# bghira/universal-metal-flash-attention

Hardware: AMD Instinct MI355X
Metric: SDPA fwd TFLOPS (bf16) + int8 speedup, B=1 H=24 S=4096 D=128, 1/2/4/8 GPU (higher is better)
Workload: dtype bf16

## Files before the change

universal-metal-flash-attention_amd/csrc/fa_fwd16_w64.hip:

```cpp
#include <algorithm>
#include <cmath>
#include <cstdlib>
#include <type_traits>

#include "fa_fwd16_w64_params.h"

namespace umfa {

#define W64_I8 0
#define W64_BODY_INC "fa_fwd16_w64_body.inc"
#define W64_T __bf16
#define W64_MFMA "v_mfma_f32_32x32x16_bf16"
#define W64_MFMA_QK "v_mfma_f32_32x32x16_bf16"
#define W64_MSUM "v_mfma_f32_4x4x4_16b_bf16"
#define W64_ONES_BITS 0x3f803f80u
#define W64_LAZY_PARTS 1
#define W64_CVT "v_cvt_pk_bf16_f32"
#define W64_KERNEL fa_fwd16_w64_bf16
#include "fa_fwd16_w64_kernel.inc"
#undef W64_T
#undef W64_MFMA
#undef W64_MFMA_QK
#undef W64_MSUM
#undef W64_ONES_BITS
// ... 317 lines not shown
        const uint64_t items = (uint64_t)p.B * p.H * ((p.Sq + 255) / 256);
        const uint64_t cus = (uint64_t)w64_cu_count();
        if (const int gi = tuning().w64_grid.load(std::memory_order_relaxed)) {
            if (gi > 0 && (uint64_t)gi <= cus && (uint64_t)gi <= items && gi <= 512) return (uint32_t)gi;
        }
        const uint64_t gmax = cus < 512 ? cus : 512;
        if (items < cus) return (uint32_t)((p.ms[2] == 0 && items * ((p.Skv + 63) / 64) >= cus * 10) ? gmax : items);
        return (uint32_t)gmax;
    }
    const bool pairs = p.causal && !w64_is_window(p);
    uint64_t total = (uint64_t)p.B * p.H * ((p.Sq + 255) / 256) * w64_tiles_per_item(p);
    if (pairs) total = (uint64_t)p.B * p.H * (((p.Sq + 255) / 256 + 1) / 2);
    const uint32_t cus = (uint32_t)w64_cu_count();
    if (const int gi = tuning().w64_grid.load(std::memory_order_relaxed)) {
        const uint32_t g = (uint32_t)gi;
        if (gi > 0 && g <= cus && g <= total) return g;
    }
    if (!pairs) {
        const uint64_t items = (uint64_t)p.B * p.H * ((p.Sq + 255) / 256);
        if (items < cus && cus / items >= 2 && items * (cus / items) <= total) return (uint32_t)(items * (cus / items));
        if (items < cus && 2 * (uint64_t)w64_tiles_per_item(p) * (cus - items) < 35 * cus) return (uint32_t)items;
    }
    return total < cus ? (uint32_t)total : cus;
}

uint32_t fwd_w64_grid(const FwdParams& p) { return w64_grid(p); }

FwdW64Plan fwd_w64_plan(const FwdParams& p) {
    FwdW64Plan plan;
    const uint32_t items = p.B * p.H * ((p.Sq + 255) / 256);
    (void)items;
    plan.cnt_bytes = ((size_t)w64_grid(p) * sizeof(uint32_t) + 255) & ~(size_t)255;
    plan.buf_bytes = (size_t)2 * w64_grid(p) * (4 * 2 * 17 * 1024);
    return plan;
}

template <typename KFN>
static hipError_t launch_w64_kernel(KFN kfn, const FwdParams& p, const W64Params& wp, hipStream_t stream) {
    const uint32_t grid = w64_grid(p);
    const size_t lds = 65536 + 4 * 32 * (512 + 16) + 64 + 4096 + 8192 + 2048 + 64;
    if (hipError_t e = ensure_dynamic_lds((const void*)kfn, lds); e != hipSuccess) return e;
    hipLaunchKernelGGL(kfn, dim3(grid), dim3(256), lds, stream, wp);
    return hipGetLastError();
}

hipError_t launch_fwd_w64(const FwdParams& p, float* part_buf, uint32_t* part_cnt, hipStream_t stream, const char** name) {
    if (!fwd_w64_supported(p) || !part_buf || !part_cnt) return hipErrorNotSupported;
    W64Params wp;
    wp.q = p.q; wp.k = p.k; wp.v = p.v; wp.o = p.o; wp.lse = p.lse;
    for (int i = 0; i < 3; ++i) { wp.qs[i] = p.qs[i]; wp.ks[i] = p.ks[i]; wp.vs[i] = p.vs[i]; }
    wp.B = p.B; wp.H = p.H; wp.Sq = p.Sq; wp.Skv = p.Skv;
    wp.scale = p.scale;
    wp.n_items = p.B * p.H * ((p.Sq + 255) / 256);
    wp.T = (p.Skv + 63) / 64;
    wp.part_buf = part_buf;
    wp.part_cnt = part_cnt;
    w64_softmax_policy(p.in_prec, &wp.tau, &wp.lazy);
    wp.skew = (uint32_t)tuning().w64_skew.load(std::memory_order_relaxed);
    if (tuning().w64_skew.load(std::memory_order_relaxed) == -1) wp.skew = 0xffffffffu;
    wp.rope_cos = p.rope_cos; wp.rope_sin = p.rope_sin; wp.rope_tb = p.rope_tb;
    wp.vsc = p.vsc; wp.vsc_bs = p.vsc_bs; wp.vsc_hs = p.vsc_hs;
    if (p.in_prec == P_BF16 && p.pv16 && !p.vsc) return hipErrorInvalidValue;
    wp.Tw = wp.T; wp.win_left = wp.win_right = 0;
    const bool rope = p.rope_cos != nullptr, window = w64_is_window(p), fp32o = p.out_prec == P_FP32, maska = p.mask_kind == MK_F16, maskt = p.mask_kind == MK_BOOL || maska;
    wp.mask = nullptr; wp.mask_s[0] = wp.mask_s[1] = wp.mask_s[2] = 0;
    wp.guard = maska ? p.guard : nullptr;
    if (p.guard && (!maska || p.guard_want != 0u)) return hipErrorInvalidValue;
    if (maskt) {
        if ((!maska && !p.mk_bits) || !p.mk_list || !p.mk_cnt) return hipErrorInvalidValue;
        if (maska) { wp.mask = p.mask; wp.mask_s[0] = p.ms[0]; wp.mask_s[1] = p.ms[1]; wp.mask_s[2] = p.ms[2]; }
        wp.mk_bits = p.mk_bits; wp.mk_list = p.mk_list; wp.mk_cnt = p.mk_cnt;
        wp.mk_bs = p.mk_bs; wp.mk_hs = p.mk_hs; wp.mk_nrb64 = p.mk_nrb64;
        wp.mk_prefix = p.mk_prefix;
#ifndef W64_LAB_MASK_FORCE_LAZY
        if (p.ms[2] != 0 || p.causal || tuning().no_w64_mask_lazy.load(std::memory_order_relaxed)) wp.lazy = 0;
#endif
    }
    if (rope && p.out_prec != p.in_prec) return hipErrorNotSupported;
    if (window) {
        wp.Tw = w64_tiles_per_item(p);
        wp.win_left = (int32_t)w64_win_left(p);
        wp.win_right = (int32_t)w64_win_right(p);
    }
#define W64_FAMILY(FAM, T16, HAS_ROPE)                                                                                         \
    do {                                                                                                                       \
        if constexpr (HAS_ROPE >= 2) {        \
            if (maskt) return fp32o ? launch_w64_kernel(FAM<float, false, false, false, true>, p, wp, stream) : launch_w64_kernel(FAM<T16, false, false, false, true>, p, wp, stream); \
        }                                                                                                                      \
        if constexpr (HAS_ROPE == 1 || HAS_ROPE == 2) {                                                                        \
            if (rope) return p.causal ? launch_w64_kernel(FAM<T16, true, true>, p, wp, stream) : launch_w64_kernel(FAM<T16, false, true>, p, wp, stream); \
        }                                                                                                                      \
        if (window) return fp32o ? launch_w64_kernel(FAM<float, false, false, true>, p, wp, stream) : launch_w64_kernel(FAM<T16, false, false, true>, p, wp, stream); \
        if (p.causal) return fp32o ? launch_w64_kernel(FAM<float, true>, p, wp, stream) : launch_w64_kernel(FAM<T16, true>, p, wp, stream); \
        return fp32o ? launch_w64_kernel(FAM<float, false>, p, wp, stream) : launch_w64_kernel(FAM<T16, false>, p, wp, stream); \
    } while (0)
    static const char* const names[3][2][3] = {
        {{"fa_fwd16_w64<bf16,128>", "fa_fwd16_w64<bf16,128,rope>", "fa_fwd16_w64<bf16,128,window>"},
         {"fa_fwd16_w64<bf16,64>", "fa_fwd16_w64<bf16,64,rope>", "fa_fwd16_w64<bf16,64,window>"}},
        {{"fa_fwd16_w64<bf16,128,pv16>", "fa_fwd16_w64<bf16,128,pv16,rope>", "fa_fwd16_w64<bf16,128,pv16,window>"},
         {"fa_fwd16_w64<bf16,64,pv16>", "fa_fwd16_w64<bf16,64,pv16,rope>", "fa_fwd16_w64<bf16,64,pv16,window>"}},
        {{"fa_fwd16_w64<fp16,128>", "fa_fwd16_w64<fp16,128,rope>", "fa_fwd16_w64<fp16,128,window>"},
         {"fa_fwd16_w64<fp16,64>", "fa_fwd16_w64<fp16,64,rope>", "fa_fwd16_w64<fp16,64,window>"}}};
    if (p.D == 64 && rope) return hipErrorNotSupported;
    const int fam = p.in_prec == P_BF16 ? (p.pv16 ? 1 : 0) : 2;
    if (maskt && fam == 0) return hipErrorNotSupported;
    if (maska && fam == 0) return hipErrorNotSupported;
    if (maska) {
        *name = p.D == 64 ? (fam == 1 ? "fa_fwd16_w64<bf16,64,pv16,bias>" : "fa_fwd16_w64<fp16,64,bias>") : (fam == 1 ? "fa_fwd16_w64<bf16,128,pv16,bias>" : "fa_fwd16_w64<fp16,128,bias>");
        return launch_fwd_w64_bias(wp, fam, fp32o, w64_grid(p), 65536 + 4 * 32 * (512 + 16) + 64 + 4096 + 8192 + 2048 + 64, stream, (int)p.D);
    }
    *name = maska ? (fam == 1 ? "fa_fwd16_w64<bf16,128,pv16,bias>" : "fa_fwd16_w64<fp16,128,bias>") : maskt ? (p.D == 64 ? (fam == 1 ? "fa_fwd16_w64<bf16,64,pv16,mask>" : "fa_fwd16_w64<fp16,64,mask>")
                               : (fam == 1 ? "fa_fwd16_w64<bf16,128,pv16,mask>" : "fa_fwd16_w64<fp16,128,mask>"))
                  : names[fam][p.D == 64 ? 1 : 0][rope ? 1 : window ? 2 : 0];
    if (p.D == 64) {
        if (fam == 0) W64_FAMILY(fa_fwd16_w64d64_bf16, __bf16, 0);
        if (fam == 1) W64_FAMILY(fa_fwd16_w64d64_bf16pv16, __bf16, 3);
        W64_FAMILY(fa_fwd16_w64d64_f16, _Float16, 3);
    }
    if (fam == 0) W64_FAMILY(fa_fwd16_w64_bf16, __bf16, 1);
    if (fam == 1) W64_FAMILY(fa_fwd16_w64_bf16pv16, __bf16, 2);
    W64_FAMILY(fa_fwd16_w64_f16, _Float16, 2);
#undef W64_FAMILY
}

bool fwd_w64_i8_supported(const FwdParams& p) {
    if (tuning().no_w64.load(std::memory_order_relaxed) || p.D != 128) return false;
    if (!(p.scale > 0.0f)) return false;
    if (p.Skv < 64 || p.Sq < 256 || (p.Sq % 256 != 0 && p.Sq < 1024)) return false;
    if (p.mask_kind == MK_BOOL && p.mask) {
        if (tuning().no_w64_mask.load(std::memory_order_relaxed) || p.causal) return false;
        if (((p.Skv + 63) / 64) > 1024u || w64_grid(p) > 512u) return false;
        if (tuning().force_w64.load(std::memory_order_relaxed)) return true;
        const uint64_t blocks = (uint64_t)p.B * p.H * ((p.Sq + 255) / 256), cus = (uint64_t)w64_cu_count();
        return blocks >= cus || (p.ms[2] == 0 && blocks * ((p.Skv + 63) / 64) >= cus * 10) || ((p.ms[0] != 0 || p.ms[1] != 0) && blocks * 8 >= cus * 3);
    }
    return p.mask_kind == MK_NONE && !p.mask;
}

hipError_t launch_fwd_w64_i8(const FwdParams& p, const QuantViews& v, float* part_buf, uint32_t* part_cnt, hipStream_t stream) {
    if (!fwd_w64_i8_supported(p) || !part_buf || !part_cnt || v.dpq != 128) return hipErrorNotSupported;
    W64I8Params wp;
    wp.q8 = v.q8; wp.k8 = v.k8; wp.v16 = (const _Float16*)v.v16;
    wp.v8 = v.v8; wp.v_e8 = v.v_e8;
    wp.q_scale = v.q_scale; wp.k_scale = v.k_scale;
    wp.o = p.o; wp.lse = p.lse;
    wp.B = p.B; wp.H = p.H; wp.Sq = p.Sq; wp.Skv = p.Skv; wp.nqblk = v.nqblk; wp.nkblk = v.nkblk;
    wp.scale = p.scale;
    wp.n_items = p.B * p.H * ((p.Sq + 255) / 256);
    wp.T = (p.Skv + 63) / 64;
    wp.part_buf = part_buf;
    wp.part_cnt = part_cnt;
    w64_softmax_policy(P_FP16, &wp.tau, &wp.lazy);
    wp.skew = (uint32_t)tuning().w64_skew.load(std::memory_order_relaxed);
    wp.vsc = v.v8 ? nullptr : p.vsc;
    const uint32_t grid = w64_grid(p);
    const bool f8 = v.v8 != nullptr, maskt = p.mask_kind == MK_BOOL;
    wp.mk_bits = wp.mk_list = wp.mk_cnt = nullptr; wp.mk_bs = wp.mk_hs = wp.mk_nrb64 = 0;
    if (maskt) {
        if (f8 || p.causal || !p.mk_bits || !p.mk_list || !p.mk_cnt) return hipErrorInvalidValue;
        wp.mk_bits = p.mk_bits; wp.mk_list = p.mk_list; wp.mk_cnt = p.mk_cnt;
        wp.mk_bs = p.mk_bs; wp.mk_hs = p.mk_hs; wp.mk_nrb64 = p.mk_nrb64;
        if (p.ms[2] != 0 || tuning().no_w64_mask_lazy.load(std::memory_order_relaxed)) wp.lazy = 0;
    }
    const size_t lds = maskt ? 65536 + 4 * 32 * (512 + 16) + 64 + 4096 + 8192 + 2048 + 64 : 65536 + 4 * 32 * (512 + 16) + 16;
    auto kfn = f8 ? (p.causal ? fa_fwd_w64_i8f8<float, true> : fa_fwd_w64_i8f8<float, false>)
                  : maskt ? fa_fwd_w64_i8<float, false, true>
                          : (p.causal ? fa_fwd_w64_i8<float, true> : fa_fwd_w64_i8<float, false>);
    if (hipError_t e = ensure_dynamic_lds((const void*)kfn, lds); e != hipSuccess) return e;
    hipLaunchKernelGGL(kfn, dim3(grid), dim3(256), lds, stream, wp);
    return hipGetLastError();
}

}
```

universal-metal-flash-attention_amd/csrc/fa_fwd16_w64_kernel.inc:

```

#ifdef W64_ABL_NOBAR
#define W64_ITER_BARRIER() asm volatile("" ::: "memory")
#elif defined(W64_LAB_WAITSTAMP)
#define W64_ITER_BARRIER()                                                                         \
    do {                                                                                           \
        asm volatile("s_waitcnt lgkmcnt(0)" ::: "memory");                                         \
        const unsigned long long w0_ = __builtin_amdgcn_s_memtime();                               \
        asm volatile("s_waitcnt vmcnt(0) lgkmcnt(0)" ::: "memory");                                \
        const unsigned long long w1_ = __builtin_amdgcn_s_memtime();                               \
        asm volatile("s_waitcnt lgkmcnt(0)\n\ts_barrier" ::: "memory");                            \
        const unsigned long long w2_ = __builtin_amdgcn_s_memtime();                               \
        asm volatile("s_waitcnt lgkmcnt(0)" ::: "memory");                                         \
        st_wait += w1_ - w0_;                                                                      \
        st_bar += w2_ - w1_;                                                                       \
    } while (0)
#elif defined(W64_ABL_VMCNT8)
#define W64_ITER_BARRIER() asm volatile("s_waitcnt vmcnt(8) lgkmcnt(0)\n\ts_barrier" ::: "memory")
#else
#define W64_ITER_BARRIER() asm volatile("s_waitcnt vmcnt(0) lgkmcnt(0)\n\ts_barrier" ::: "memory")
#endif
#ifdef W64_ABL_NODMA
#define W64_DMA_ON 0
#else
#define W64_DMA_ON 1
// ... 138 lines not shown
    auto v_frag = [&](int voff, int db, int st) -> V8 {
        const V4 lo = tr_read_at(vtr[db] + (unsigned)(voff + (16 * st) * ROW_IN));
        const V4 hi4 = tr_read_at(vtr[db] + (unsigned)(voff + (16 * st + 8) * ROW_IN));
        return __builtin_shufflevector(lo, hi4, 0, 1, 2, 3, 4, 5, 6, 7);
    };
    (void)v_frag;

#if W64_F8
    typedef int i32x8 __attribute__((ext_vector_type(8)));
    const unsigned v8addr = lds0 + (unsigned)lane * 16u;
    auto v8_frag = [&](int voff, int db) -> i32x8 {
        const i32x4 lo = *(const i32x4 LDS_AS*)(uintptr_t)(v8addr + (unsigned)(voff + db * 2048));
        const i32x4 hi4 = *(const i32x4 LDS_AS*)(uintptr_t)(v8addr + (unsigned)(voff + db * 2048 + 1024));
        return __builtin_shufflevector(lo, hi4, 0, 1, 2, 3, 4, 5, 6, 7);
    };
#endif

#if W64_I8
    const int k_stride_b = 128, v_stride_b = 256, q_stride_b = 128;
#else
    const int k_stride_b = (int)p.ks[2] * 2, v_stride_b = (int)p.vs[2] * 2, q_stride_b = (int)p.qs[2] * 2;
#endif
    int kdma0[4], vdma0[4];
    {
        constexpr int RPI = 1024 / ROW_IN, CPR = ROW_IN / 16, PPW = 16 / RPI;
        const int d_r = lane / CPR, d_c = lane % CPR;
        (void)d_c;
#pragma unroll
        for (int j = 0; j < 4; ++j) {
            const int row = (uw * PPW + (j % PPW)) * RPI + d_r;
            (void)row;
#if W64_F8
            vdma0[j] = ((uw * 2 + (j & 1)) * 64 + lane) * 16;
#else
            vdma0[j] = row * v_stride_b + (v_off<W64_DP>(row, d_c) - row * ROW_IN);
#endif
#if W64_I8
            const int krow = (uw * 2 + (j & 1)) * 8 + (lane >> 3), kc = lane & 7;
            kdma0[j] = krow * 128 + (k8_off_128(krow, kc) - krow * 128);
#else
            kdma0[j] = row * k_stride_b + (k_off<W64_DP>(row, d_c) - row * ROW_IN);
#endif
        }
    }
    const int k_step0 = 64 * k_stride_b, v_step0 = W64_F8 ? 8192 : 64 * v_stride_b;
    const unsigned lds_wave = __builtin_amdgcn_readfirstlane(lds0 + (unsigned)uw * (W64_F8 ? 2048u : (unsigned)(16 * ROW_IN)));
#if W64_I8
    const unsigned lds_wave_k = __builtin_amdgcn_readfirstlane(lds0 + (unsigned)uw * 2048u);
    float c2 = 0.0f;
#ifndef W64_I8_NOBIAS
    constexpr float I8_BIAS = 12582912.0f;
#if W64_F8
    f8_init_consts();
#else
    i8_init_bias();
#endif
    float nmb[2] = {0.f, 0.f};
#endif
#else
    const unsigned lds_wave_k = lds_wave;
    const float c2 = p.scale * UMFA_LOG2E;
#endif

    const uint32_t G = gridDim.x;
    const uint32_t w = xcd_remap(blockIdx.x, G);
    const uint32_t T_ = p.T;
    const uint32_t nqb = (p.Sq + 255) / 256;
    const bool ktail = (p.Skv & 63) != 0;
    const uint32_t jobs_per_head = (nqb + 1) / 2, n_jobs = p.B * p.H * jobs_per_head;
    uint32_t Tst = T_;
    int win_left = 0, win_right = 0;
#if !W64_I8
    if constexpr (WINDOW) { Tst = p.Tw; win_left = p.win_left; win_right = p.win_right; }
#endif
    (void)win_left; (void)win_right;
    constexpr bool SPARSE = CAUSAL || WINDOW || MASKT;
    auto mk_slab = [&](uint32_t bh_) -> uint32_t { return (bh_ / p.H) * p.mk_bs + (bh_ % p.H) * p.mk_hs; };
    auto item_tiles = [&](uint32_t item) -> uint32_t {
        if constexpr (MASKT) return p.mk_cnt[mk_slab(item / nqb) * nqb + item % nqb];
        if constexpr (!CAUSAL) return Tst;
        const uint32_t q = item % nqb;
        return 4 * q + 4 < T_ ? 4 * q + 4 : T_;
    };
    const bool whole_rem = !CAUSAL && p.skew == 0xffffffffu;
    const uint32_t full_rounds = CAUSAL ? 0u : whole_rem ? (p.n_items + G - 1) / G : p.n_items / G;
    const uint32_t rem_items = (CAUSAL || whole_rem) ? 0u : p.n_items - full_rounds * G;
    constexpr unsigned MK_PREFIX_OFF = 65536u + 4u * 32u * (512u + 16u) + 64u + 4096u + 8192u;
    if constexpr (MASKT) {
        if (rem_items) {
            volatile uint32_t* const pf = (volatile uint32_t*)(smem + MK_PREFIX_OFF);
            const uint32_t first = full_rounds * G, j0 = threadIdx.x, j1 = threadIdx.x + 256u;
            for (uint32_t j = threadIdx.x; j < rem_items; j += 256u) {
                const uint32_t it_ = first + j;
                pf[1 + j] = p.mk_cnt[mk_slab(it_ / nqb) * nqb + it_ % nqb];
            }
            if (threadIdx.x == 0) pf[0] = 0u;
            __syncthreads();
            for (uint32_t off = 1; off < rem_items; off <<= 1) {
                const uint32_t a0 = (j0 < rem_items && j0 >= off) ? pf[1 + j0 - off] : 0u;
                const uint32_t a1 = (j1 < rem_items && j1 >= off) ? pf[1 + j1 - off] : 0u;
                __syncthreads();
                if (j0 < rem_items) pf[1 + j0] += a0;
                if (j1 < rem_items) pf[1 + j1] += a1;
                __syncthreads();
            }
        }
    }
    auto mk_prefix_at = [&](uint32_t j) -> uint32_t {
        return (uint32_t)__builtin_amdgcn_readfirstlane((int)((volatile const uint32_t*)(smem + MK_PREFIX_OFF))[j]);
    };
    (void)mk_prefix_at;
    auto item_start = [&](uint32_t litem) -> uint64_t {
        if constexpr (MASKT) return mk_prefix_at(litem);
        return (uint64_t)litem * Tst;
    };
    auto item_of_step = [&](uint64_t step) -> uint32_t {
        if constexpr (MASKT) {
            uint32_t lo = 0, hi_ = rem_items - 1;
            while (lo < hi_) {
                const uint32_t mid = (lo + hi_ + 1) >> 1;
                if (mk_prefix_at(mid) <= step) lo = mid; else hi_ = mid - 1;
            }
            return lo;
        }
        return (uint32_t)(step / Tst);
    };
    const uint64_t total = MASKT ? (rem_items ? (uint64_t)mk_prefix_at(rem_items) : 0ull) : (uint64_t)rem_items * Tst;
    const uint32_t skew = (!MASKT && rem_items && G == 2 * rem_items && p.skew != 0xffffffffu && 2 * p.skew < Tst) ? p.skew : 0u;
    const uint32_t Gs = (MASKT && total < G) ? (uint32_t)total : G;
    auto slice_bound = [&](uint32_t g) -> uint32_t {
        if constexpr (MASKT) { if (g >= Gs) return (uint32_t)total; }
        return (uint32_t)(total * g / Gs) - ((g & 1u) ? skew : 0u);
    };
    const uint32_t s_begin = slice_bound(w), s_end = slice_bound(w + 1);
#ifdef W64_LAB_GAPSTAMP
    unsigned long long st_g[4] = {0, 0, 0, 0}, st_gprev = 0;
#define W64_GSTAMP(k)                                                                            \
    do {                                                                                         \
        asm volatile("s_waitcnt lgkmcnt(0)" ::: "memory");                                       \
        const unsigned long long now_ = __builtin_amdgcn_s_memtime();                            \
        asm volatile("s_waitcnt lgkmcnt(0)" ::: "memory");                                       \
        if (st_gprev) st_g[k] += now_ - st_gprev;                                                \
        st_gprev = now_;                                                                         \
    } while (0)
#endif
#ifdef W64_LAB_FSTAMP
    unsigned long long fs_now[8] = {0, 0, 0, 0, 0, 0, 0, 0};
    uint32_t fs_acc[8] = {0, 0, 0, 0, 0, 0, 0, 0}, fs_last = 0, fs_tiles = 0;
    bool fs_valid = false;
#define W64_FSTAMP(k) asm volatile("s_memtime %0" : "=s"(fs_now[k]))
#define W64_FSTAMP_END(n)                                                                           \
    do {                                                                                            \
        asm volatile("s_waitcnt lgkmcnt(0)" ::: "memory");                                          \
        if (fs_valid) fs_acc[0] += (uint32_t)fs_now[0] - fs_last;                                   \
        _Pragma("unroll") for (int k_ = 1; k_ < (n); ++k_) fs_acc[k_] += (uint32_t)fs_now[k_] - (uint32_t)fs_now[k_ - 1]; \
        fs_last = (uint32_t)fs_now[(n) - 1];                                                        \
        fs_valid = true;                                                                            \
        ++fs_tiles;                                                                                 \
    } while (0)
#endif
#ifdef W64_LAB_STAMPS
    const unsigned long long st_rt0 = __builtin_amdgcn_s_memrealtime(), st_ck0 = __builtin_amdgcn_s_memtime();
    unsigned long long st_pro = 0, st_loop = 0, st_drain = 0, st_epi = 0, st_t = 0, st_wait = 0, st_bar = 0;
#define W64_STAMP(acc) do { const unsigned long long now_ = __builtin_amdgcn_s_memtime(); acc += now_ - st_t; st_t = now_; } while (0)
#else
#define W64_STAMP(acc) do { } while (0)
#endif

    uint32_t ntail = 0;
    bool tail_first = false;
    if (s_end > s_begin) {
        const uint32_t it0 = item_of_step(s_begin), it1 = item_of_step(s_end - 1);
        ntail = it1 - it0 + 1;
        tail_first = item_start(it0) != s_begin;
    }
    const uint32_t my_jobs = CAUSAL ? (n_jobs > w ? (n_jobs - w + G - 1) / G : 0u) : 0u;
    const uint32_t nseg = CAUSAL ? 2 * my_jobs : full_rounds + ntail;

    auto make_srd = [&](const void* base, uint32_t bytes) {
        const unsigned long long a = (unsigned long long)base;
        i32x4 d;
        d[0] = __builtin_amdgcn_readfirstlane((int)(a & 0xffffffffu));
        d[1] = __builtin_amdgcn_readfirstlane((int)((a >> 32) & 0xffffu));
        d[2] = __builtin_amdgcn_readfirstlane((int)bytes);
        d[3] = 0x00020000;
        return d;
    };
    auto seg_decode = [&](uint32_t si_, uint32_t& item_, uint32_t& t0_, uint32_t& n_, uint32_t& litem_, bool& desc_) -> bool {
        litem_ = 0;
        desc_ = false;
        if constexpr (CAUSAL) {
            const uint32_t job = (si_ >> 1) * G + w, jbh = job / jobs_per_head, jj = job % jobs_per_head;
            desc_ = (si_ & 1) != 0;
            const uint32_t q = desc_ ? nqb - 1 - jj : jj;
            if (desc_ && q == jj) return false;
            item_ = jbh * nqb + q;
            t0_ = 0;
            n_ = item_tiles(item_);
        } else {
            const bool is_tail = tail_first ? (si_ < ntail) : (si_ >= full_rounds);
            if (is_tail) {
                const uint32_t ti = tail_first ? si_ : si_ - full_rounds;
                litem_ = item_of_step(s_begin) + ti;
                const uint64_t ist = item_start(litem_), ien = MASKT ? item_start(litem_ + 1) : ist + Tst;
                const uint64_t sb = ist > s_begin ? ist : s_begin, se = ien < s_end ? ien : s_end;
                t0_ = (uint32_t)(sb - ist);
                n_ = (uint32_t)(se - sb);
                item_ = full_rounds * G + litem_;
            } else {
                item_ = (tail_first ? si_ - ntail : si_) * G + w;
                if (item_ >= p.n_items) return false;
                t0_ = 0;
                n_ = MASKT ? item_tiles(item_) : Tst;
            }
        }
// ... 564 lines not shown
            dmask[0] += dm_step;
            dmask[1] += dm_step;
            if constexpr (WINDOW) dleft += dm_step;
            W64_END_ITER(0, true, fix_e_b);
            }
#undef W64_KOFF
#undef W64_KNEXT
#undef W64_VOFF
#undef W64_KDST
#undef W64_VDST
#undef W64_MOFF
#undef W64_MDST
            ++i;
            if (i >= n) { last_a = false; break; }
#define W64_KOFF 0
#define W64_KNEXT KSLOT
#define W64_VOFF (VRING + VSLOT)
#define W64_KDST KSLOT
#define W64_VDST VRING
#define W64_MOFF 0u
#define W64_MDST 8192u
            mk_steps(i);
            mk_request(i + 1, mk_next);
#if W64_I8
            c2 = W64_C2(sq * k_scale_of(tile_at(i)));
            W64_SET_NMB();
            W64_SET_VSC(tile_at(i - 1));
#endif
#if W64_LAZY_PARTS
            if (lazy) {
                if (W64_MASKED_TILE(i)) {
                    mk_take(i);
#define W64_PART 11
#include W64_BODY_INC
#undef W64_PART
                } else {
#define W64_PART 9
#include W64_BODY_INC
#undef W64_PART
                }
                dmask[0] += dm_step;
                dmask[1] += dm_step;
                if constexpr (WINDOW) dleft += dm_step;
                W64_END_ITER_LAZY(KSLOT, fix_e_a);
            } else
#endif
            {
            if (W64_MASKED_TILE(i)) {
                mk_take(i);
#define W64_PART 7
#include W64_BODY_INC
#undef W64_PART
            } else {
#define W64_PART 2
#include W64_BODY_INC
#undef W64_PART
            }
            dmask[0] += dm_step;
            dmask[1] += dm_step;
            if constexpr (WINDOW) dleft += dm_step;
            W64_END_ITER(KSLOT, true, fix_e_a);
            }
#undef W64_KOFF
#undef W64_KNEXT
#undef W64_VOFF
#undef W64_KDST
#undef W64_VDST
#undef W64_MOFF
#undef W64_MDST
            ++i;
        }
        W64_STAMP(st_loop);
#if W64_PREFETCH_NEXT
        if constexpr (!ROPE_ON) {
            uint32_t sj = si + 1, it_ = 0, t0_ = 0, n_ = 0, li_ = 0;
            bool d_ = false;
            while (sj < nseg && !seg_decode(sj, it_, t0_, n_, li_, d_)) ++sj;
            if (sj < nseg) {
                issue_q_k0(it_, d_ ? n_ - 1 : t0_, d_ ? -k_step0 : k_step0);
                have_pref = true;
            }
        }
#endif
        W64_SET_VSC(tile_at(n - 1));
        if (last_a) {
#define W64_VOFF VRING
#define W64_PART 3
#include W64_BODY_INC
#undef W64_PART
#undef W64_VOFF
        } else {
#define W64_VOFF (VRING + VSLOT)
#define W64_PART 4
#include W64_BODY_INC
#undef W64_PART
#undef W64_VOFF
        }
#undef W64_DECIDE
#undef W64_UNBIAS
#undef W64_SET_NMB
#undef W64_MGRID
#undef W64_C2
#undef W64_END_ITER
#ifdef W64_END_ITER_LAZY
#undef W64_END_ITER_LAZY
#undef W64_LAZY_QUICK
#endif
#undef W64_DECIDE2
#undef W64_MOVE_REF
#undef W64_NOFIX
#undef W64_SCALE_LACC
#undef W64_SET_VSC
        asm volatile("s_nop 15\n\ts_nop 15");

        W64_STAMP(st_drain);
        float lt[2];
#if W64_F8
        f8_read_l(lt[0], lt[1]);
#else
        W64_L_READ(lt[0], lt[1]);
#if W64_LAZY_PARTS
        if (lazy_on) {
            const unsigned flag_at = lds0 + OVF_FLAG_OFF;
            ovf = ovf || __builtin_amdgcn_ballot_w64(!(lt[0] < LAZY_OVF) | !(lt[1] < LAZY_OVF)) != 0;
            if constexpr (SPARSE) {
                const uint32_t ta = tile_at(0), tb = tile_at(n - 1);
                const int64_t klo = 64 * (int64_t)(ta < tb ? ta : tb);
                int64_t khi = 64 * (int64_t)(ta < tb ? tb : ta) + 63;
                khi = khi < (int64_t)p.Skv - 1 ? khi : (int64_t)p.Skv - 1;
                bool lost = false;
#pragma unroll
                for (int qb = 0; qb < 2; ++qb) {
                    const int64_t row = (int64_t)q0 + 32 * qb + ql;
                    const int64_t lo = WINDOW ? (klo > row - win_left ? klo : row - win_left) : klo;
                    const int64_t hi_k = WINDOW ? (khi < row + win_right ? khi : row + win_right) : (khi < row ? khi : row);
                    lost |= lo <= hi_k && !(lt[qb] + xor32(lt[qb]) > LAZY_LOST);
                }
                ovf = ovf || __builtin_amdgcn_ballot_w64(lost) != 0;
            }
            if (lazy && ovf && lane == 0) *(volatile uint32_t LDS_AS*)(uintptr_t)flag_at = 1u;
            asm volatile("s_waitcnt lgkmcnt(0)\n\ts_barrier" ::: "memory");
            const uint32_t redo = *(volatile uint32_t LDS_AS*)(uintptr_t)flag_at;
            asm volatile("s_waitcnt lgkmcnt(0)\n\ts_barrier" ::: "memory");
            if (redo) {
                if (tid == 0) *(volatile uint32_t LDS_AS*)(uintptr_t)flag_at = 0u;
                force_exact = true;
#if W64_PREFETCH_NEXT
                have_pref = false;
#endif
                --si;
                continue;
            }
        }
#endif
        lt[0] += xor32(lt[0]);
        lt[1] += xor32(lt[1]);
#endif

#ifndef W64_VSC
#define W64_VSC 0
#endif
#if W64_VSC == 2
        const float vsc = p.vsc ? p.vsc[128 * (size_t)bh + 65] : 1.0f;
#elif W64_VSC
        const float vsc = p.vsc[128 * ((size_t)b * p.vsc_bs + (size_t)h * p.vsc_hs) + 65];
#else
        constexpr float vsc = 1.0f;
#endif
        constexpr int ROWB = (W64_I8 ? 128 : W64_DP) * (int)sizeof(OUT), STG_STRIDE = ROWB + 16;
        const unsigned stg = lds0 + 65536u + (unsigned)uw * (32 * (512 + 16));
        int ql_e = ql;
        if constexpr (MASKA) asm volatile("" : "+v"(ql_e));
        auto stage_block = [&](int db, const float (&ob)[16], float inv) {
#pragma unroll
            for (int g = 0; g < 4; ++g) {
                const unsigned a = stg + (unsigned)(ql_e * STG_STRIDE + (32 * db + 8 * g + 4 * hi) * (int)sizeof(OUT));
                if constexpr (sizeof(OUT) == 4) {
                    *(f32x4 LDS_AS*)(uintptr_t)a = f32x4{ob[4 * g] * inv, ob[4 * g + 1] * inv, ob[4 * g + 2] * inv, ob[4 * g + 3] * inv};
                } else {
                    typedef OUT O4 __attribute__((ext_vector_type(4)));
                    *(O4 LDS_AS*)(uintptr_t)a = O4{(OUT)(ob[4 * g] * inv), (OUT)(ob[4 * g + 1] * inv), (OUT)(ob[4 * g + 2] * inv),
                                                   (OUT)(ob[4 * g + 3] * inv)};
                }
            }
        };
        auto flush_rows = [&](int qb) {
            constexpr int CPR = ROWB / 16, RPI = 64 / CPR;
            char* __restrict__ ob = (char*)p.o + ((int64_t)bh * p.Sq + q0 + 32 * qb) * ROWB;
#pragma unroll
            for (int it = 0; it < 32 / RPI; ++it) {
                const int row = it * RPI + lane / CPR, ch = lane % CPR;
                const u32x4_t v = *(const u32x4_t LDS_AS*)(uintptr_t)(stg + (unsigned)(row * STG_STRIDE + ch * 16));
#ifdef W64_ABL_NOSTORE
                if (q0 + 32 * qb + row < p.Sq && p.Sq == 0xffffffffu) *(u32x4_t*)(ob + row * ROWB + ch * 16) = v;
#elif defined(W64_LAB_NT_STORE)
                if (q0 + 32 * qb + row < p.Sq) __builtin_nontemporal_store(v, (u32x4_t*)(ob + row * ROWB + ch * 16));
#else
                if (q0 + 32 * qb + row < p.Sq) *(u32x4_t*)(ob + row * ROWB + ch * 16) = v;
#endif
            }
        };

        if (n == Ti) {
            auto out_qb = [&](auto QBC) {
                constexpr int qb = decltype(QBC)::value;
                const uint32_t q_row = q0 + 32 * qb + ql;
                const float inv = ((WINDOW || MASKT) && !(lt[qb] > 0.0f)) ? 0.0f : (1.0f / lt[qb]) * vsc;
                auto one_db = [&](auto DBC) {
                    constexpr int db = decltype(DBC)::value;
                    float ob[16];
                    if constexpr (qb == 0) read_o0<db>(ob); else read_o1<db>(ob);
                    stage_block(db, ob, inv);
                };
                one_db(std::integral_constant<int, 0>{});
                one_db(std::integral_constant<int, 1>{});
                if constexpr (W64_I8 || W64_DP == 128) {
                    one_db(std::integral_constant<int, 2>{});
                    one_db(std::integral_constant<int, 3>{});
                }
                flush_rows(qb);
                if (p.lse && hi == 0 && q_row < p.Sq) p.lse[(int64_t)bh * p.Sq + q_row] = (mr[qb] + log2f(lt[qb])) * UMFA_LN2;
            };
            out_qb(std::integral_constant<int, 0>{});
            out_qb(std::integral_constant<int, 1>{});
            continue;
        }

#ifdef W64_ABL_NOCOMBINE
        continue;
#endif
        auto owner_of = [&](uint64_t step) -> uint32_t {
            uint32_t g = (uint32_t)((step * Gs) / total);
            while (g + 1 < Gs && slice_bound(g + 1) <= step) ++g;
            while (g > 0 && slice_bound(g) > step) --g;
            return g;
        };
        const uint32_t w_first = owner_of(item_start(litem));
        const uint32_t w_last = owner_of(item_start(litem) + Ti - 1);
        const uint32_t nparts = w_last - w_first + 1, j_own = w - w_first;
        constexpr uint32_t SLOT_B = 4 * 2 * 17 * 1024;
        int lane_f = lane;
        if constexpr (MASKA) asm volatile("" : "+v"(lane_f));
        auto slot_off = [&](uint32_t j) -> uint32_t {
            const uint32_t sl = j == 0 ? 2 * w_first + 1 : 2 * (w_first + j);
            return sl * SLOT_B + (uint32_t)uw * (2 * 17 * 1024) + (uint32_t)lane_f * 16;
        };
        const auto prsrc = __builtin_amdgcn_make_buffer_rsrc((void*)p.part_buf, 0, (int)(2 * G * SLOT_B), 0x00020000);
        volatile uint32_t* flag_s = (volatile uint32_t*)(smem + 65536 + 4 * 32 * (512 + 16) + 4);
        asm volatile("s_barrier" ::: "memory");
        if (tid == 0) flag_s[0] = __hip_atomic_load(p.part_cnt + litem, __ATOMIC_RELAXED, __HIP_MEMORY_SCOPE_AGENT);
        __syncthreads();
        bool folder = flag_s[0] == nparts - 1;
        if (!folder) {
            const uint32_t mine = slot_off(j_own);
            auto publish_qb = [&](auto QBC) {
                constexpr int qb = decltype(QBC)::value;
                auto pub_db = [&](auto DBC) {
                    constexpr int db = decltype(DBC)::value;
                    float ob[16];
                    if constexpr (qb == 0) read_o0<db>(ob); else read_o1<db>(ob);
#pragma unroll
                    for (int g = 0; g < 4; ++g)
                        __builtin_amdgcn_raw_buffer_store_b128(
                            __builtin_bit_cast(u32x4_t, f32x4{ob[4 * g], ob[4 * g + 1], ob[4 * g + 2], ob[4 * g + 3]}), prsrc,
                            (int)(mine + (qb * 17 + db * 4 + g) * 1024), 0, 16);
                };
                pub_db(std::integral_constant<int, 0>{});
                pub_db(std::integral_constant<int, 1>{});
                if constexpr (W64_I8 || W64_DP == 128) {
                    pub_db(std::integral_constant<int, 2>{});
                    pub_db(std::integral_constant<int, 3>{});
                }
                __builtin_amdgcn_raw_buffer_store_b128(__builtin_bit_cast(u32x4_t, f32x4{lt[qb] > 0.0f ? mr[qb] : -INFINITY, lt[qb], 0.0f, 0.0f}), prsrc,
                                                       (int)(mine + (qb * 17 + 16) * 1024), 0, 16);
            };
            publish_qb(std::integral_constant<int, 0>{});
            publish_qb(std::integral_constant<int, 1>{});
            asm volatile("s_waitcnt vmcnt(0)" ::: "memory");
            __syncthreads();
            if (tid == 0) flag_s[1] = __hip_atomic_fetch_add(p.part_cnt + litem, 1u, __ATOMIC_RELAXED, __HIP_MEMORY_SCOPE_AGENT);
            __syncthreads();
            folder = flag_s[1] == nparts - 1;
        }
        if (!folder) continue;
        if (tid == 0) __hip_atomic_store(p.part_cnt + litem, 0u, __ATOMIC_RELAXED, __HIP_MEMORY_SCOPE_AGENT);
        __builtin_amdgcn_fence(__ATOMIC_ACQUIRE, "wavefront");

        auto fold_qb = [&](auto QBC) {
            constexpr int qb = decltype(QBC)::value;
            const float m_own = lt[qb] > 0.0f ? mr[qb] : -INFINITY;
            float mm = m_own;
            for (uint32_t j = 0; j < nparts; ++j) {
                if (j == j_own) continue;
                const f32x4 ml = __builtin_bit_cast(f32x4, __builtin_amdgcn_raw_buffer_load_b128(prsrc, (int)(slot_off(j) + (qb * 17 + 16) * 1024), 0, 16));
                mm = fmaxf(mm, ml[0]);
            }
            float ll = 0.0f;
            const uint32_t q_row = q0 + 32 * qb + ql;
            auto fold_half = [&](auto HC) {
                constexpr int h2 = decltype(HC)::value;
                float acc[32];
#pragma unroll
                for (int r = 0; r < 32; ++r) acc[r] = 0.0f;
                float lsum = 0.0f;
                for (uint32_t j = 0; j < nparts; ++j) {
                    float x[32], mj, lj;
                    if (j == j_own) {
                        float t0[16], t1[16];
                        if constexpr (qb == 0) { read_o0<2 * h2>(t0); read_o0<2 * h2 + 1>(t1); } else { read_o1<2 * h2>(t0); read_o1<2 * h2 + 1>(t1); }
#pragma unroll
                        for (int r = 0; r < 16; ++r) { x[r] = t0[r]; x[16 + r] = t1[r]; }
                        mj = m_own;
                        lj = lt[qb];
                    } else {
                        const uint32_t so = slot_off(j) + qb * 17 * 1024;
                        f32x4 c[8];
#pragma unroll
                        for (int k = 0; k < 8; ++k)
                            c[k] = __builtin_bit_cast(f32x4, __builtin_amdgcn_raw_buffer_load_b128(prsrc, (int)(so + (8 * h2 + k) * 1024), 0, 16));
                        const f32x4 ml = __builtin_bit_cast(f32x4, __builtin_amdgcn_raw_buffer_load_b128(prsrc, (int)(so + 16 * 1024), 0, 16));
#pragma unroll
                        for (int k = 0; k < 8; ++k)
#pragma unroll
                            for (int e = 0; e < 4; ++e) x[4 * k + e] = c[k][e];
                        mj = ml[0];
                        lj = ml[1];
                    }
                    const float wj = (SPARSE && mj == -INFINITY) ? 0.0f : __builtin_amdgcn_exp2f(mj - mm);
                    lsum += wj * lj;
#pragma unroll
                    for (int r = 0; r < 32; ++r) acc[r] += wj * x[r];
                }
                ll = lsum;
                const float inv = ((WINDOW || MASKT) && !(lsum > 0.0f)) ? 0.0f : (1.0f / lsum) * vsc;
                float b0[16], b1[16];
#pragma unroll
                for (int r = 0; r < 16; ++r) { b0[r] = acc[r]; b1[r] = acc[16 + r]; }
                stage_block(2 * h2, b0, inv);
                stage_block(2 * h2 + 1, b1, inv);
            };
            fold_half(std::integral_constant<int, 0>{});
            if constexpr (W64_I8 || W64_DP == 128) fold_half(std::integral_constant<int, 1>{});
            flush_rows(qb);
            if (p.lse && hi == 0 && q_row < p.Sq) p.lse[(int64_t)bh * p.Sq + q_row] = (mm + log2f(ll)) * UMFA_LN2;
        };
        fold_qb(std::integral_constant<int, 0>{});
        fold_qb(std::integral_constant<int, 1>{});
    }
#ifdef W64_LAB_STAMPS
    asm volatile("s_waitcnt vmcnt(0)" ::: "memory");
    W64_STAMP(st_epi);
    asm volatile("s_barrier" ::: "memory");
    if (tid == 0 && p.lse) {
        unsigned long long* dbg = (unsigned long long*)p.lse + (size_t)blockIdx.x * 8;
        dbg[4] = st_pro;
        dbg[5] = st_loop;
#if defined(W64_LAB_FSTAMP)
        dbg[4] = ((unsigned long long)fs_acc[1] << 32) | fs_acc[0];
        dbg[5] = ((unsigned long long)fs_acc[3] << 32) | fs_acc[2];
        dbg[6] = ((unsigned long long)fs_acc[5] << 32) | fs_acc[4];
        dbg[7] = ((unsigned long long)fs_acc[7] << 32) | fs_acc[6];
        (void)st_wait; (void)st_bar; (void)fs_tiles;
#elif defined(W64_LAB_GAPSTAMP)
        dbg[4] = st_g[0]; dbg[5] = st_g[1];
        dbg[6] = st_g[2];
        dbg[7] = st_g[3];
        (void)st_wait; (void)st_bar;
#elif defined(W64_LAB_WAITSTAMP) || defined(W64_LAB_DMASTAMP)
        dbg[6] = st_wait;
        dbg[7] = st_bar;
#else
        (void)st_wait; (void)st_bar;
        dbg[6] = st_drain;
        dbg[7] = st_epi;
#endif
        dbg[0] = st_rt0;
        dbg[1] = __builtin_amdgcn_s_memrealtime();
        dbg[2] = st_ck0;
        dbg[3] = __builtin_amdgcn_s_memtime();
    }
#endif
}
#ifdef W64_L_ZERO
#undef W64_L_ZERO
#undef W64_L_SCALE
#undef W64_L_READ
#endif
#undef W64_NVGPR
```

universal-metal-flash-attention_amd/csrc/fa_fwd16_w64_params.h:

```cpp
#pragma once
#include <cstdint>

#include "fa_common.h"
#include "fa_fwd_16_kernel.h"
#include "kernels.h"

namespace umfa {

struct W64Params {
    const void* q;
    const void* k;
    const void* v;
    void* o;
    float* lse;
    int64_t qs[3], ks[3], vs[3];
    uint32_t B, H, Sq, Skv;
    float scale;
    uint32_t n_items, T;
    float* part_buf;
    uint32_t* part_cnt;
    float tau;
    uint32_t lazy;
    uint32_t skew;
    uint32_t Tw;
    int32_t win_left, win_right;
    const float* rope_cos;
    const float* rope_sin;
    int64_t rope_tb;
    const uint32_t* mk_bits;
    const uint32_t* mk_list;
    const uint32_t* mk_cnt;
    uint32_t mk_bs, mk_hs, mk_nrb64;
    const uint32_t* mk_prefix;
    const void* mask;
    int64_t mask_s[3];
    const float* vsc;
    uint32_t vsc_bs, vsc_hs;
    const uint32_t* guard;
};

#include "fa_fwd16_w64_regs.inc"

__device__ __forceinline__ constexpr int k8_off_128(int row, int ch) { return row * 128 + 16 * (ch ^ ((row >> 1) & 7)); }

struct W64I8Params {
    const int8_t* q8;
    const int8_t* k8;
    const _Float16* v16;
    const uint8_t* v8;
    const uint32_t* v_e8;
    const float* q_scale;
    const float* k_scale;
    void* o;
    float* lse;
    uint32_t B, H, Sq, Skv, nqblk, nkblk;
    float scale;
    uint32_t n_items, T;
    float* part_buf;
    uint32_t* part_cnt;
    float tau;
    uint32_t lazy;
    uint32_t skew;
    const uint32_t* mk_bits;
    const uint32_t* mk_list;
    const uint32_t* mk_cnt;
    uint32_t mk_bs, mk_hs, mk_nrb64;
    const float* vsc;
};

hipError_t launch_fwd_w64_bias(const W64Params& wp, int family, bool fp32_out, uint32_t grid, size_t lds, hipStream_t stream, int head_dim);

}
```

Measured before the change: 1062.

## Precompute W64 split schedule on host and pipeline two-part partial fold

Moves the full-round, remainder and skew schedule computation from the kernel onto the host launch path, and uses 32-bit division in slice/owner computation when it fits. The partial-completion counter is loaded early so its latency overlaps the V drain. It also adds a specialized fold path for the common two-part split-K case that issues the other partial's loads ahead of use in double-buffered stages. A batched max pass is added for the general case. This adds register pressure and code size in the epilogue.

```diff
diff --git a/universal-metal-flash-attention_amd/csrc/fa_fwd16_w64.hip b/universal-metal-flash-attention_amd/csrc/fa_fwd16_w64.hip
--- a/universal-metal-flash-attention_amd/csrc/fa_fwd16_w64.hip
+++ b/universal-metal-flash-attention_amd/csrc/fa_fwd16_w64.hip
@@ -423,6 +423,7 @@
         wp.win_left = (int32_t)w64_win_left(p);
         wp.win_right = (int32_t)w64_win_right(p);
     }
+    w64_schedule(wp, w64_grid(p), wp.Tw);
 #define W64_FAMILY(FAM, T16, HAS_ROPE)                                                                                         \
     do {                                                                                                                       \
         if constexpr (HAS_ROPE >= 2) {        \
@@ -495,6 +496,7 @@
     wp.skew = (uint32_t)tuning().w64_skew.load(std::memory_order_relaxed);
     wp.vsc = v.v8 ? nullptr : p.vsc;
     const uint32_t grid = w64_grid(p);
+    w64_schedule(wp, grid, wp.T);
     const bool f8 = v.v8 != nullptr, maskt = p.mask_kind == MK_BOOL;
     wp.mk_bits = wp.mk_list = wp.mk_cnt = nullptr; wp.mk_bs = wp.mk_hs = wp.mk_nrb64 = 0;
     if (maskt) {
diff --git a/universal-metal-flash-attention_amd/csrc/fa_fwd16_w64_kernel.inc b/universal-metal-flash-attention_amd/csrc/fa_fwd16_w64_kernel.inc
--- a/universal-metal-flash-attention_amd/csrc/fa_fwd16_w64_kernel.inc
+++ b/universal-metal-flash-attention_amd/csrc/fa_fwd16_w64_kernel.inc
@@ -244,9 +244,8 @@
         const uint32_t q = item % nqb;
         return 4 * q + 4 < T_ ? 4 * q + 4 : T_;
     };
-    const bool whole_rem = !CAUSAL && p.skew == 0xffffffffu;
-    const uint32_t full_rounds = CAUSAL ? 0u : whole_rem ? (p.n_items + G - 1) / G : p.n_items / G;
-    const uint32_t rem_items = (CAUSAL || whole_rem) ? 0u : p.n_items - full_rounds * G;
+    const uint32_t full_rounds = CAUSAL ? 0u : p.sch_rounds;
+    const uint32_t rem_items = CAUSAL ? 0u : p.sch_rem;
     constexpr unsigned MK_PREFIX_OFF = 65536u + 4u * 32u * (512u + 16u) + 64u + 4096u + 8192u;
     if constexpr (MASKT) {
         if (rem_items) {
@@ -288,11 +287,14 @@
         return (uint32_t)(step / Tst);
     };
     const uint64_t total = MASKT ? (rem_items ? (uint64_t)mk_prefix_at(rem_items) : 0ull) : (uint64_t)rem_items * Tst;
-    const uint32_t skew = (!MASKT && rem_items && G == 2 * rem_items && p.skew != 0xffffffffu && 2 * p.skew < Tst) ? p.skew : 0u;
+    const uint32_t skew = (MASKT || CAUSAL) ? 0u : p.sch_skew;
     const uint32_t Gs = (MASKT && total < G) ? (uint32_t)total : G;
+    const bool div32 = ((total * G) >> 32) == 0;
     auto slice_bound = [&](uint32_t g) -> uint32_t {
+        if constexpr (CAUSAL) return 0u;
         if constexpr (MASKT) { if (g >= Gs) return (uint32_t)total; }
-        return (uint32_t)(total * g / Gs) - ((g & 1u) ? skew : 0u);
+        const uint32_t q = div32 ? (uint32_t)total * g / Gs : (uint32_t)(total * g / Gs);
+        return q - ((g & 1u) ? skew : 0u);
     };
     const uint32_t s_begin = slice_bound(w), s_end = slice_bound(w + 1);
 #ifdef W64_LAB_GAPSTAMP
@@ -1023,6 +1025,8 @@
             }
         }
 #endif
+        uint32_t tick_early = 0;
+        if (n != Ti && tid == 0) tick_early = __hip_atomic_load(p.part_cnt + litem, __ATOMIC_RELAXED, __HIP_MEMORY_SCOPE_AGENT);
         W64_SET_VSC(tile_at(n - 1));
         if (last_a) {
 #define W64_VOFF VRING
@@ -1055,6 +1059,9 @@
         asm volatile("s_nop 15\n\ts_nop 15");
 
         W64_STAMP(st_drain);
+        int tid_x = tid;
+        asm volatile("" : "+v"(tid_x));
+        const int lane_x = tid_x & 63, ql_x = lane_x & 31, hi_x = lane_x >> 5;
         float lt[2];
 #if W64_F8
         f8_read_l(lt[0], lt[1]);
@@ -1110,12 +1117,12 @@
 #endif
         constexpr int ROWB = (W64_I8 ? 128 : W64_DP) * (int)sizeof(OUT), STG_STRIDE = ROWB + 16;
         const unsigned stg = lds0 + 65536u + (unsigned)uw * (32 * (512 + 16));
-        int ql_e = ql;
+        int ql_e = ql_x;
         if constexpr (MASKA) asm volatile("" : "+v"(ql_e));
         auto stage_block = [&](int db, const float (&ob)[16], float inv) {
 #pragma unroll
             for (int g = 0; g < 4; ++g) {
-                const unsigned a = stg + (unsigned)(ql_e * STG_STRIDE + (32 * db + 8 * g + 4 * hi) * (int)sizeof(OUT));
+                const unsigned a = stg + (unsigned)(ql_e * STG_STRIDE + (32 * db + 8 * g + 4 * hi_x) * (int)sizeof(OUT));
                 if constexpr (sizeof(OUT) == 4) {
                     *(f32x4 LDS_AS*)(uintptr_t)a = f32x4{ob[4 * g] * inv, ob[4 * g + 1] * inv, ob[4 * g + 2] * inv, ob[4 * g + 3] * inv};
                 } else {
@@ -1130,7 +1137,7 @@
             char* __restrict__ ob = (char*)p.o + ((int64_t)bh * p.Sq + q0 + 32 * qb) * ROWB;
 #pragma unroll
             for (int it = 0; it < 32 / RPI; ++it) {
-                const int row = it * RPI + lane / CPR, ch = lane % CPR;
+                const int row = it * RPI + lane_x / CPR, ch = lane_x % CPR;
                 const u32x4_t v = *(const u32x4_t LDS_AS*)(uintptr_t)(stg + (unsigned)(row * STG_STRIDE + ch * 16));
 #ifdef W64_ABL_NOSTORE
                 if (q0 + 32 * qb + row < p.Sq && p.Sq == 0xffffffffu) *(u32x4_t*)(ob + row * ROWB + ch * 16) = v;
@@ -1145,7 +1152,7 @@
         if (n == Ti) {
             auto out_qb = [&](auto QBC) {
                 constexpr int qb = decltype(QBC)::value;
-                const uint32_t q_row = q0 + 32 * qb + ql;
+                const uint32_t q_row = q0 + 32 * qb + ql_x;
                 const float inv = ((WINDOW || MASKT) && !(lt[qb] > 0.0f)) ? 0.0f : (1.0f / lt[qb]) * vsc;
                 auto one_db = [&](auto DBC) {
                     constexpr int db = decltype(DBC)::value;
@@ -1160,7 +1167,7 @@
                     one_db(std::integral_constant<int, 3>{});
                 }
                 flush_rows(qb);
-                if (p.lse && hi == 0 && q_row < p.Sq) p.lse[(int64_t)bh * p.Sq + q_row] = (mr[qb] + log2f(lt[qb])) * UMFA_LN2;
+                if (p.lse && hi_x == 0 && q_row < p.Sq) p.lse[(int64_t)bh * p.Sq + q_row] = (mr[qb] + log2f(lt[qb])) * UMFA_LN2;
             };
             out_qb(std::integral_constant<int, 0>{});
             out_qb(std::integral_constant<int, 1>{});
@@ -1171,7 +1178,7 @@
         continue;
 #endif
         auto owner_of = [&](uint64_t step) -> uint32_t {
-            uint32_t g = (uint32_t)((step * Gs) / total);
+            uint32_t g = div32 ? (uint32_t)step * Gs / (uint32_t)total : (uint32_t)((step * Gs) / total);
             while (g + 1 < Gs && slice_bound(g + 1) <= step) ++g;
             while (g > 0 && slice_bound(g) > step) --g;
             return g;
@@ -1180,7 +1187,7 @@
         const uint32_t w_last = owner_of(item_start(litem) + Ti - 1);
         const uint32_t nparts = w_last - w_first + 1, j_own = w - w_first;
         constexpr uint32_t SLOT_B = 4 * 2 * 17 * 1024;
-        int lane_f = lane;
+        int lane_f = lane_x;
         if constexpr (MASKA) asm volatile("" : "+v"(lane_f));
         auto slot_off = [&](uint32_t j) -> uint32_t {
             const uint32_t sl = j == 0 ? 2 * w_first + 1 : 2 * (w_first + j);
@@ -1189,7 +1196,7 @@
         const auto prsrc = __builtin_amdgcn_make_buffer_rsrc((void*)p.part_buf, 0, (int)(2 * G * SLOT_B), 0x00020000);
         volatile uint32_t* flag_s = (volatile uint32_t*)(smem + 65536 + 4 * 32 * (512 + 16) + 4);
         asm volatile("s_barrier" ::: "memory");
-        if (tid == 0) flag_s[0] = __hip_atomic_load(p.part_cnt + litem, __ATOMIC_RELAXED, __HIP_MEMORY_SCOPE_AGENT);
+        if (tid == 0) flag_s[0] = tick_early;
         __syncthreads();
         bool folder = flag_s[0] == nparts - 1;
         if (!folder) {
@@ -1227,17 +1234,117 @@
         if (tid == 0) __hip_atomic_store(p.part_cnt + litem, 0u, __ATOMIC_RELAXED, __HIP_MEMORY_SCOPE_AGENT);
         __builtin_amdgcn_fence(__ATOMIC_ACQUIRE, "wavefront");
 
+        constexpr int NH = (W64_I8 || W64_DP == 128) ? 2 : 1;
+        const float m_own[2] = {lt[0] > 0.0f ? mr[0] : -INFINITY, lt[1] > 0.0f ? mr[1] : -INFINITY};
+        auto fold_add = [&](float (&acc)[32], float& lsum, const float (&x)[32], float mj, float lj, float mm) {
+            const float wj = (SPARSE && mj == -INFINITY) ? 0.0f : __builtin_amdgcn_exp2f(mj - mm);
+            lsum += wj * lj;
+#pragma unroll
+            for (int r = 0; r < 32; ++r) acc[r] += wj * x[r];
+        };
+        auto own_half = [&](auto QBC, auto HC, float (&x)[32]) {
+            constexpr int qb = decltype(QBC)::value, h2 = decltype(HC)::value;
+            float t0[16], t1[16];
+            if constexpr (qb == 0) { read_o0<2 * h2>(t0); read_o0<2 * h2 + 1>(t1); } else { read_o1<2 * h2>(t0); read_o1<2 * h2 + 1>(t1); }
+#pragma unroll
+            for (int r = 0; r < 16; ++r) { x[r] = t0[r]; x[16 + r] = t1[r]; }
+        };
+        auto fold_finish = [&](int qb, int h2, const float (&acc)[32], float lsum, float mm) {
+            const float inv = ((WINDOW || MASKT) && !(lsum > 0.0f)) ? 0.0f : (1.0f / lsum) * vsc;
+            float b0[16], b1[16];
+#pragma unroll
+            for (int r = 0; r < 16; ++r) { b0[r] = acc[r]; b1[r] = acc[16 + r]; }
+            stage_block(2 * h2, b0, inv);
+            stage_block(2 * h2 + 1, b1, inv);
+            if (h2 == NH - 1) {
+                flush_rows(qb);
+                const uint32_t q_row = q0 + 32 * qb + ql_x;
+                if (p.lse && hi_x == 0 && q_row < p.Sq) p.lse[(int64_t)bh * p.Sq + q_row] = (mm + log2f(lsum)) * UMFA_LN2;
+            }
+        };
+#ifndef W64_FOLD_PIPE
+#define W64_FOLD_PIPE 1
+#endif
+        if constexpr (W64_FOLD_PIPE != 0) {
+            if (nparts == 2) {
+                const uint32_t so = slot_off(1u - j_own);
+                auto ld = [&](int qb, int c) {
+                    return __builtin_bit_cast(f32x4, __builtin_amdgcn_raw_buffer_load_b128(prsrc, (int)(so + (uint32_t)(qb * 17 + c) * 1024u), 0, 16));
+                };
+                auto request = [&](f32x4 (&buf)[8], int s) {
+#pragma unroll
+                    for (int k = 0; k < 8; ++k) buf[k] = ld(s / NH, 8 * (s % NH) + k);
+                };
+                const f32x4 ml0 = ld(0, 16), ml1 = ld(1, 16);
+                f32x4 buf_a[8], buf_b[8];
+                request(buf_a, 0);
+                request(buf_b, 1);
+                auto fold_stage = [&](auto SC, f32x4 (&buf)[8]) {
+                    constexpr int s = decltype(SC)::value, qb = s / NH, h2 = s % NH;
+                    const f32x4 ml = qb == 0 ? ml0 : ml1;
+                    const float mm = fmaxf(m_own[qb], ml[0]);
+                    float acc[32], lsum = 0.0f;
+#pragma unroll
+                    for (int r = 0; r < 32; ++r) acc[r] = 0.0f;
+                    auto add_own = [&]() {
+                        float x[32];
+                        own_half(std::integral_constant<int, qb>{}, std::integral_constant<int, h2>{}, x);
+                        fold_add(acc, lsum, x, m_own[qb], lt[qb], mm);
+                    };
+                    auto add_other = [&]() {
+                        float x[32];
+#pragma unroll
+                        for (int k = 0; k < 8; ++k)
+#pragma unroll
+                            for (int e = 0; e < 4; ++e) x[4 * k + e] = buf[k][e];
+                        fold_add(acc, lsum, x, ml[0], ml[1], mm);
+                    };
+                    if (j_own == 0) { add_own(); add_other(); } else { add_other(); add_own(); }
+                    if constexpr (s + 2 < 2 * NH) request(buf, s + 2);
+                    fold_finish(qb, h2, acc, lsum, mm);
+                };
+                fold_stage(std::integral_constant<int, 0>{}, buf_a);
+                fold_stage(std::integral_constant<int, 1>{}, buf_b);
+                if constexpr (NH == 2) {
+                    fold_stage(std::integral_constant<int, 2>{}, buf_a);
+                    fold_stage(std::integral_constant<int, 3>{}, buf_b);
+                }
+                continue;
+            }
+        }
+        float mm2[2] = {m_own[0], m_own[1]};
+        if constexpr (W64_FOLD_PIPE != 0) {
+            for (uint32_t j0 = 0; j0 < nparts; j0 += 4) {
+                float mv[4][2];
+#pragma unroll
+                for (uint32_t u = 0; u < 4; ++u) {
+                    const uint32_t j = j0 + u, jr = (j < nparts && j != j_own) ? j : j_own;
+                    const uint32_t so = slot_off(jr);
+#pragma unroll
+                    for (int qb = 0; qb < 2; ++qb)
+                        mv[u][qb] = __builtin_bit_cast(f32x4, __builtin_amdgcn_raw_buffer_load_b128(prsrc, (int)(so + (uint32_t)(qb * 17 + 16) * 1024u), 0, 16))[0];
+                }
+#pragma unroll
+                for (uint32_t u = 0; u < 4; ++u) {
+                    const uint32_t j = j0 + u;
+                    if (j < nparts && j != j_own) {
+                        mm2[0] = fmaxf(mm2[0], mv[u][0]);
+                        mm2[1] = fmaxf(mm2[1], mv[u][1]);
+                    }
+                }
+            }
+        } else {
+#pragma unroll
+            for (int qb = 0; qb < 2; ++qb)
+                for (uint32_t j = 0; j < nparts; ++j) {
+                    if (j == j_own) continue;
+                    const f32x4 ml = __builtin_bit_cast(f32x4, __builtin_amdgcn_raw_buffer_load_b128(prsrc, (int)(slot_off(j) + (qb * 17 + 16) * 1024), 0, 16));
+                    mm2[qb] = fmaxf(mm2[qb], ml[0]);
+                }
+        }
         auto fold_qb = [&](auto QBC) {
             constexpr int qb = decltype(QBC)::value;
-            const float m_own = lt[qb] > 0.0f ? mr[qb] : -INFINITY;
-            float mm = m_own;
-            for (uint32_t j = 0; j < nparts; ++j) {
-                if (j == j_own) continue;
-                const f32x4 ml = __builtin_bit_cast(f32x4, __builtin_amdgcn_raw_buffer_load_b128(prsrc, (int)(slot_off(j) + (qb * 17 + 16) * 1024), 0, 16));
-                mm = fmaxf(mm, ml[0]);
-            }
-            float ll = 0.0f;
-            const uint32_t q_row = q0 + 32 * qb + ql;
+            const float mm = mm2[qb];
             auto fold_half = [&](auto HC) {
                 constexpr int h2 = decltype(HC)::value;
                 float acc[32];
@@ -1247,11 +1354,8 @@
                 for (uint32_t j = 0; j < nparts; ++j) {
                     float x[32], mj, lj;
                     if (j == j_own) {
-                        float t0[16], t1[16];
-                        if constexpr (qb == 0) { read_o0<2 * h2>(t0); read_o0<2 * h2 + 1>(t1); } else { read_o1<2 * h2>(t0); read_o1<2 * h2 + 1>(t1); }
-#pragma unroll
-                        for (int r = 0; r < 16; ++r) { x[r] = t0[r]; x[16 + r] = t1[r]; }
-                        mj = m_own;
+                        own_half(QBC, HC, x);
+                        mj = m_own[qb];
                         lj = lt[qb];
                     } else {
                         const uint32_t so = slot_off(j) + qb * 17 * 1024;
@@ -1267,23 +1371,12 @@
                         mj = ml[0];
                         lj = ml[1];
                     }
-                    const float wj = (SPARSE && mj == -INFINITY) ? 0.0f : __builtin_amdgcn_exp2f(mj - mm);
-                    lsum += wj * lj;
-#pragma unroll
-                    for (int r = 0; r < 32; ++r) acc[r] += wj * x[r];
+                    fold_add(acc, lsum, x, mj, lj, mm);
                 }
-                ll = lsum;
-                const float inv = ((WINDOW || MASKT) && !(lsum > 0.0f)) ? 0.0f : (1.0f / lsum) * vsc;
-                float b0[16], b1[16];
-#pragma unroll
-                for (int r = 0; r < 16; ++r) { b0[r] = acc[r]; b1[r] = acc[16 + r]; }
-                stage_block(2 * h2, b0, inv);
-                stage_block(2 * h2 + 1, b1, inv);
+                fold_finish(qb, h2, acc, lsum, mm);
             };
             fold_half(std::integral_constant<int, 0>{});
-            if constexpr (W64_I8 || W64_DP == 128) fold_half(std::integral_constant<int, 1>{});
-            flush_rows(qb);
-            if (p.lse && hi == 0 && q_row < p.Sq) p.lse[(int64_t)bh * p.Sq + q_row] = (mm + log2f(ll)) * UMFA_LN2;
+            if constexpr (NH == 2) fold_half(std::integral_constant<int, 1>{});
         };
         fold_qb(std::integral_constant<int, 0>{});
         fold_qb(std::integral_constant<int, 1>{});
diff --git a/universal-metal-flash-attention_amd/csrc/fa_fwd16_w64_params.h b/universal-metal-flash-attention_amd/csrc/fa_fwd16_w64_params.h
--- a/universal-metal-flash-attention_amd/csrc/fa_fwd16_w64_params.h
+++ b/universal-metal-flash-attention_amd/csrc/fa_fwd16_w64_params.h
@@ -22,6 +22,7 @@
     float tau;
     uint32_t lazy;
     uint32_t skew;
+    uint32_t sch_rounds, sch_rem, sch_skew;
     uint32_t Tw;
     int32_t win_left, win_right;
     const float* rope_cos;
@@ -38,6 +39,14 @@
     uint32_t vsc_bs, vsc_hs;
     const uint32_t* guard;
 };
+
+template <typename P>
+inline void w64_schedule(P& wp, uint32_t grid, uint32_t steps) {
+    const bool whole_rem = wp.skew == 0xffffffffu;
+    wp.sch_rounds = whole_rem ? (wp.n_items + grid - 1) / grid : wp.n_items / grid;
+    wp.sch_rem = whole_rem ? 0u : wp.n_items - wp.sch_rounds * grid;
+    wp.sch_skew = (wp.sch_rem && grid == 2 * wp.sch_rem && !whole_rem && 2 * (uint64_t)wp.skew < steps) ? wp.skew : 0u;
+}
 
 #include "fa_fwd16_w64_regs.inc"
 
@@ -61,6 +70,7 @@
     float tau;
     uint32_t lazy;
     uint32_t skew;
+    uint32_t sch_rounds, sch_rem, sch_skew;
     const uint32_t* mk_bits;
     const uint32_t* mk_list;
     const uint32_t* mk_cnt;
```

Result: no change. 1068, median of 6 (+0.6%).
